# amathislab/BUCTD

Measured on AMD Instinct MI355X. Metric: images/sec (train) BUCTD-CoAM-W48 384x288, higher is better.
Workload: dtype f32 (3x3 convs: operands split exactly into 3 bf16 pieces, 6 bf16 MFMAs per product, fp32 accumulate - fp32-class); 1 GPU; BUCTD-CoAM-W48 (pose_hrnet_coam, ATT_MODULES [F,T,F,F], colored condition) 384x288 CrowdPose-14kpt full train step: fwd + JointsMSE + bwd + grad all-reduce + Adam + arg-max accuracy decode; global_batch=32, batch_per_gpu=32, input=N x 6 x 384 x 288 fp32, params=115581770, parallelism=dp1, hip_streams=4, conv_math=bf16x6, step_graph=False

## Files before the change

buctd_amd/csrc/conv3x3_wgrad.hip:

```cpp
#include "c3_common.h"

typedef __bf16 bf16x4 __attribute__((ext_vector_type(4)));

#define WG_MAX_SW 75
#define WG_PRO 96

template <int NP> struct WGeo;
template <> struct WGeo<2> { static constexpr int KB = 96; };
template <> struct WGeo<3> { static constexpr int KB = 64; };

struct WG3Args {
  const float* x;
  const float* dy;
  float* part;
  int N, H, W, Ci, Co;
  int SW, IB, P;
  int split_q, split_rem;
  const float* x_mean;
  const float* x_invstd;
  const float* x_gamma;
  const float* x_beta;
  int x_relu;
  unsigned ib_mul, ib_sh, sw_mul, sw_sh;
};

__device__ __forceinline__ int wg_fast_div(int n, unsigned mul, unsigned sh) {
  return (int)(__umulhi((unsigned)n, mul) >> sh);
}

typedef float wg_f32x2 __attribute__((ext_vector_type(2)));
typedef __bf16 wg_bf16x2 __attribute__((ext_vector_type(2)));
typedef unsigned wg_u32x2 __attribute__((ext_vector_type(2)));
template <int NP, int LO>
__device__ __forceinline__ void wg_split_store(unsigned char* row, int c, f32x4 v) {
  wg_f32x2 lo = {v.x, v.y}, hi = {v.z, v.w};
#pragma unroll
  for (int q = 0; q < NP; ++q) {
    const unsigned a = __builtin_bit_cast(unsigned, __builtin_convertvector(lo, wg_bf16x2));
    const unsigned b = __builtin_bit_cast(unsigned, __builtin_convertvector(hi, wg_bf16x2));
    *reinterpret_cast<wg_u32x2*>(row + q * LO + 2 * c) = (wg_u32x2){a, b};
    if (q + 1 < NP) {
      lo -= (wg_f32x2){__uint_as_float(a << 16), __uint_as_float(a & 0xffff0000u)};
      hi -= (wg_f32x2){__uint_as_float(b << 16), __uint_as_float(b & 0xffff0000u)};
    }
  }
}

__device__ __forceinline__ bf16x8 tr_frag(const unsigned char* p, int row_bytes) {
  typedef __attribute__((address_space(3))) bf16x4 lds_bf16x4;
  const bf16x4 a = __builtin_amdgcn_ds_read_tr16_b64_v4bf16((lds_bf16x4*)p);
  const bf16x4 b = __builtin_amdgcn_ds_read_tr16_b64_v4bf16((lds_bf16x4*)(p + 4 * row_bytes));
  return __builtin_shufflevector(a, b, 0, 1, 2, 3, 4, 5, 6, 7);
}

__device__ __forceinline__ bf16x8 tr_frag2(const unsigned char* p, const unsigned char* q) {
  typedef __attribute__((address_space(3))) bf16x4 lds_bf16x4;
  const bf16x4 a = __builtin_amdgcn_ds_read_tr16_b64_v4bf16((lds_bf16x4*)p);
  const bf16x4 b = __builtin_amdgcn_ds_read_tr16_b64_v4bf16((lds_bf16x4*)q);
  return __builtin_shufflevector(a, b, 0, 1, 2, 3, 4, 5, 6, 7);
}

__device__ __forceinline__ int ring_slot(int r, int ring) {
  return r - (r >= ring ? ring : 0);
}

#define WG_OOB 0x80000000u
template <int NP, int CF>
__device__ __forceinline__ void wg3_tile(const WG3Args& p, unsigned char* smem, int bxc, int byc, int z, int ncx, int nz) {
  constexpr int KB = WGeo<NP>::KB;
  constexpr int CH = CF * 16;
  constexpr int LO = CH * 2;
  constexpr int RS = (CH * 2 * NP) % 64 == 32 ? CH * 2 * NP : CH * 2 * NP + 32;
  constexpr int C4 = CH / 4;
  constexpr int PD = (KB * C4 + 255) / 256;
  constexpr int PP = (WG_PRO * C4 + 255) / 256;
  constexpr int NFR = 9 * CF;
  constexpr int NW = (NFR + 3) / 4;
  constexpr bool WHOLE = KB * C4 == PD * 256;

  const int R = KB + 2 * p.SW + 2;
  unsigned char* Dt = smem;
  unsigned char* Xt = smem + (size_t)KB * RS;
  float* bntab = reinterpret_cast<float*>(Xt + (size_t)R * RS);

  const int t = threadIdx.x, lane = t & 63;
  const int wave = __builtin_amdgcn_readfirstlane(t >> 6);
  const int t16 = lane & 15, g = lane >> 4;
  const int co0 = bxc * CH, ci0 = byc * CH;
  const int k_begin = (z * p.split_q + (z < p.split_rem ? z : p.split_rem)) * KB;
  int k_end = k_begin + (p.split_q + (z < p.split_rem ? 1 : 0)) * KB;
  if (k_end > p.P) k_end = p.P;
  const int halo = p.SW + 1;
  const int ci_lim = p.Ci - ci0;
  const bool x_bn = p.x_mean != nullptr;

  const __amdgpu_buffer_rsrc_t r_x = __builtin_amdgcn_make_buffer_rsrc(const_cast<float*>(p.x), 0, (unsigned)p.N * p.H * p.W * p.Ci * 4u, 0x00020000);
  const __amdgpu_buffer_rsrc_t r_d = __builtin_amdgcn_make_buffer_rsrc(const_cast<float*>(p.dy), 0, (unsigned)p.N * p.H * p.W * p.Co * 4u, 0x00020000);
  typedef unsigned wg_u32x4 __attribute__((ext_vector_type(4)));
  auto bload = [&](__amdgpu_buffer_rsrc_t r, unsigned off) -> f32x4 {
    return __builtin_bit_cast(f32x4, __builtin_amdgcn_raw_buffer_load_b128(r, off, 0, 0));
  };
  auto pos_offset = [&](int pp, int C, bool ok) -> unsigned {
    const int n = wg_fast_div(pp, p.ib_mul, p.ib_sh);
    const int rem = pp - n * p.IB;
    const int yy = wg_fast_div(rem, p.sw_mul, p.sw_sh);
    const int xx = rem - yy * p.SW;
    const bool real = ok & (pp >= 0) & (pp < p.P) & (n < p.N) & (yy >= 1) & (xx >= 1) & (xx <= p.W);
    return real ? (unsigned)(((n * p.H + yy - 1) * p.W + xx - 1) * C) * 4u : WG_OOB;
  };
  int srow[PD], sc4[PD];
#pragma unroll
  for (int q = 0; q < PD; ++q) {
    const int idx = t + 256 * q;
    srow[q] = idx / C4;
    sc4[q] = (idx - srow[q] * C4) * 4;
  }
  auto bn_in = [&](f32x4 v, int c, bool real) -> f32x4 {
    const f32x4 mu = *reinterpret_cast<const f32x4*>(bntab + c);
    const f32x4 sc = *reinterpret_cast<const f32x4*>(bntab + CH + c);
    const f32x4 be = *reinterpret_cast<const f32x4*>(bntab + 2 * CH + c);
#pragma unroll
    for (int j = 0; j < 4; ++j) {
      const float u = (v[j] - mu[j]) * sc[j] + be[j];
      const float w = p.x_relu ? fmaxf(u, 0.f) : u;
      v[j] = real ? w : 0.f;
    }
    return v;
  };

  f32x4 dreg[PD], xreg[PD];
  unsigned xoff[PD];
  auto load_d = [&](int k0) {
#pragma unroll
    for (int q = 0; q < PD; ++q) {
      const int pp = k0 + srow[q];
      dreg[q] = bload(r_d, pos_offset(pp, p.Co, (WHOLE || srow[q] < KB) & (pp < k_end)) + (unsigned)(co0 + sc4[q]) * 4u);
    }
  };
  auto load_x = [&](int rel0) {
#pragma unroll
    for (int q = 0; q < PD; ++q) {
      xoff[q] = pos_offset(k_begin - halo + rel0 + srow[q], p.Ci, (WHOLE || srow[q] < KB) & (sc4[q] < ci_lim));
      xreg[q] = bload(r_x, xoff[q] + (unsigned)(ci0 + sc4[q]) * 4u);
    }
  };
  auto store_d = [&]() {
#pragma unroll
    for (int q = 0; q < PD; ++q)
      if (WHOLE || srow[q] < KB) wg_split_store<NP, LO>(Dt + (size_t)srow[q] * RS, sc4[q], dreg[q]);
  };
  auto store_x = [&](int slot0) {
#pragma unroll
    for (int q = 0; q < PD; ++q)
      if (WHOLE || srow[q] < KB)
        wg_split_store<NP, LO>(Xt + (size_t)ring_slot(slot0 + srow[q], R) * RS, sc4[q],
                               x_bn ? bn_in(xreg[q], sc4[q], xoff[q] != WG_OOB) : xreg[q]);
  };

  f32x4 acc[CF][NW];
#pragma unroll
  for (int mf = 0; mf < CF; ++mf)
#pragma unroll
    for (int j = 0; j < NW; ++j) acc[mf][j] = (f32x4){0.f, 0.f, 0.f, 0.f};

  const int lane_row = g * 4 + (t16 >> 2), lane_col = (t16 & 3) * 8;
  const int lane_off = lane_row * RS + lane_col;

  if (x_bn) {
    for (int c = t; c < CH; c += 256) {
      const bool in = c < ci_lim;
      bntab[c] = in ? p.x_mean[ci0 + c] : 0.f;
      bntab[CH + c] = in ? p.x_invstd[ci0 + c] * p.x_gamma[ci0 + c] : 0.f;
      bntab[2 * CH + c] = in ? p.x_beta[ci0 + c] : 0.f;
    }
    __syncthreads();
  }
  if (k_begin < k_end) {
    const int pro = R - KB;
    for (int r0 = 0; r0 < pro; r0 += WG_PRO) {
      f32x4 preg[PP];
      unsigned poff[PP];
#pragma unroll
      for (int q = 0; q < PP; ++q) {
        const int idx = t + 256 * q;
        const int row = idx / C4, c4 = (idx - row * C4) * 4;
        poff[q] = pos_offset(k_begin - halo + r0 + row, p.Ci, (row < WG_PRO) & (r0 + row < pro) & (c4 < ci_lim));
        preg[q] = bload(r_x, poff[q] + (unsigned)(ci0 + c4) * 4u);
      }
#pragma unroll
      for (int q = 0; q < PP; ++q) {
        const int idx = t + 256 * q;
        const int row = idx / C4, c4 = (idx - row * C4) * 4;
        if (row < WG_PRO && r0 + row < pro)
          wg_split_store<NP, LO>(Xt + (size_t)(r0 + row) * RS, c4, x_bn ? bn_in(preg[q], c4, poff[q] != WG_OOB) : preg[q]);
      }
    }
    load_d(k_begin);
    load_x(pro);
  }
  int slot_new = R - KB;
  int slot_base = 0;
  int rel_next = R;
  const bool has_last = wave + 4 * (NW - 1) < NFR;
  for (int k0 = k_begin; k0 < k_end; k0 += KB) {
    __syncthreads();
    store_d();
    store_x(slot_new);
    if (k0 + KB < k_end) {
      load_d(k0 + KB);
      load_x(rel_next);
    }
    slot_new = ring_slot(slot_new + KB, R);
    rel_next += KB;
    __syncthreads();
    const unsigned ringb = (unsigned)R * RS;
    bf16x8 b[2][NP];
    auto read_b = [&](int ks, int j, bf16x8 (&dst)[NP]) {
      const int nf = wave + 4 * j;
      const int tap = nf / CF, cf = nf - tap * CF;
      const int shift = (tap / 3) * p.SW + tap % 3 + ks * 32;
      const int s = ring_slot(slot_base + shift, R);
      unsigned o0 = (unsigned)lane_off + (unsigned)(s * RS + cf * 32);
      o0 = o0 - ringb < o0 ? o0 - ringb : o0;
      unsigned o1 = o0 + 16 * RS;
      o1 = o1 - ringb < o1 ? o1 - ringb : o1;
      const unsigned char* q0 = Xt + o0;
      const unsigned char* q1 = Xt + o1;
#pragma unroll
      for (int pc = 0; pc < NP; ++pc) dst[pc] = tr_frag2(q0 + pc * LO, q1 + pc * LO);
    };
    read_b(0, 0, b[0]);
#pragma unroll
    for (int ks = 0; ks < KB / 32; ++ks) {
      bf16x8 a[NP][CF];
#pragma unroll
      for (int mf = 0; mf < CF; ++mf) {
        const unsigned char* q = Dt + (size_t)ks * 32 * RS + lane_off + mf * 32;
#pragma unroll
        for (int pc = 0; pc < NP; ++pc) a[pc][mf] = tr_frag(q + pc * LO, 4 * RS);
      }
#pragma unroll
      for (int j = 0; j < NW; ++j) {
        const int i = ks * NW + j;
        const bool more = i + 1 < (KB / 32) * NW;
        if (more) {
          const int jn = j + 1 < NW ? j + 1 : 0, ksn = j + 1 < NW ? ks : ks + 1;
          if (jn < NW - 1 || has_last) read_b(ksn, jn, b[(i + 1) & 1]);
        }
        if (j < NW - 1 || has_last) {
          bf16x8 (&bb)[NP] = b[i & 1];
#define WG_MMA(qa, qb)                                                                                      \
  _Pragma("unroll") for (int mf = 0; mf < CF; ++mf) acc[mf][j] =                                            \
      __builtin_amdgcn_mfma_f32_16x16x32_bf16(a[qa][mf], bb[qb], acc[mf][j], 0, 0, 0);
          if constexpr (NP == 3) {
            WG_MMA(2, 0) WG_MMA(0, 2) WG_MMA(1, 1) WG_MMA(1, 0) WG_MMA(0, 1) WG_MMA(0, 0)
          } else {
            WG_MMA(1, 0) WG_MMA(0, 1) WG_MMA(0, 0)
          }
#undef WG_MMA
        }
      }
    }
    slot_base = ring_slot(slot_base + KB, R);
  }

  {
    const size_t slab4 = (size_t)4 * NW * CF * 64;
    const size_t pair = (size_t)byc * ncx + bxc;
    f32x4* outp = reinterpret_cast<f32x4*>(p.part) + (pair * nz + z) * slab4;
#pragma unroll
    for (int j = 0; j < NW; ++j)
#pragma unroll
      for (int mf = 0; mf < CF; ++mf) {
        outp[((wave * NW + j) * CF + mf) * 64 + lane] = acc[mf][j];
      }
  }
}

template <int NP, int CF>
__global__ __launch_bounds__(256, 2) void conv3x3_wgrad_split_kernel(WG3Args p) {
  extern __shared__ __attribute__((aligned(16))) unsigned char smem[];
  wg3_tile<NP, CF>(p, smem, blockIdx.x, blockIdx.y, blockIdx.z, gridDim.x, gridDim.z);
}

#define WG3G_MAX 4
struct WG3Group {
  WG3Args conv[WG3G_MAX];
  int n;
  unsigned first[WG3G_MAX + 1];
  int ncx[WG3G_MAX], ncy[WG3G_MAX], nsplit[WG3G_MAX];
};
template <int NP, int CF>
__global__ __launch_bounds__(256, 2) void conv3x3_wgrad_group_kernel(WG3Group g_) {
  extern __shared__ __attribute__((aligned(16))) unsigned char smem[];
  const WG3Group& g = *(const WG3Group*)__builtin_amdgcn_kernarg_segment_ptr();
  int k = 0;
  while (k + 1 < g.n && blockIdx.x >= g.first[k + 1]) ++k;
  const unsigned lid = blockIdx.x - g.first[k], total = g.first[k + 1] - g.first[k];
  const unsigned xcd = lid & 7, idx = lid >> 3, per = total >> 3, rem = total & 7;
  const unsigned L = xcd < rem ? xcd * (per + 1) + idx : rem * (per + 1) + (xcd - rem) * per + idx;
  const unsigned pairs = (unsigned)(g.ncx[k] * g.ncy[k]);
  const unsigned z = L / pairs, pr = L - z * pairs;
  const unsigned byc = pr / (unsigned)g.ncx[k], bxc = pr - byc * (unsigned)g.ncx[k];
  wg3_tile<NP, CF>(g.conv[k], smem, (int)bxc, (int)byc, (int)z, g.ncx[k], g.nsplit[k]);
}

struct WG3Red { const float* part; float* out; int Ci, Co, nsplit, accumulate; };
template <int CF>
__device__ __forceinline__ void wg3_reduce_body(const WG3Red& a, f32x4 (&sm)[16][16], int bx, int nbx, int pair) {
  constexpr int NFR = 9 * CF;
  constexpr int NW = (NFR + 3) / 4;
  constexpr int SLAB = 4 * NW * CF * 64;
  const float* __restrict__ part = a.part;
  float* __restrict__ out = a.out;
  const int Ci = a.Ci, Co = a.Co, nsplit = a.nsplit, accumulate = a.accumulate;
  const int col = threadIdx.x & 15, zl = threadIdx.x >> 4;
  const int nco = Co / (CF * 16);
  const int co0 = (pair % nco) * CF * 16, ci0 = (pair / nco) * CF * 16;
  const f32x4* base = reinterpret_cast<const f32x4*>(part) + (size_t)pair * nsplit * SLAB;
  for (int e0 = bx * 16; e0 < SLAB; e0 += nbx * 16) {
    const int e = e0 + col;
    f32x4 s0 = (f32x4){0.f, 0.f, 0.f, 0.f}, s1 = s0, s2 = s0, s3 = s0;
    if (e < SLAB) {
      const f32x4* src = base + e;
      int zz = zl;
      for (; zz + 48 < nsplit; zz += 64) {
        s0 += src[(size_t)zz * SLAB];
        s1 += src[(size_t)(zz + 16) * SLAB];
        s2 += src[(size_t)(zz + 32) * SLAB];
        s3 += src[(size_t)(zz + 48) * SLAB];
      }
      for (; zz < nsplit; zz += 16) s0 += src[(size_t)zz * SLAB];
    }
    sm[zl][col] = (s0 + s1) + (s2 + s3);
    __syncthreads();
    if (zl == 0 && e < SLAB) {
      f32x4 sv = sm[0][col];
#pragma unroll
      for (int k = 1; k < 16; ++k) sv += sm[k][col];
      const int lane = e & 63, r = e >> 6;
      const int mf = r % CF, wj = r / CF, j = wj % NW, wv = wj / NW;
      const int nf = wv + 4 * j;
      if (nf < NFR) {
        const int tap = nf / CF, cf = nf - tap * CF;
        const int ci = ci0 + cf * 16 + (lane & 15);
        if (ci < Ci)
#pragma unroll
        for (int rg = 0; rg < 4; ++rg) {
          const int co = co0 + mf * 16 + (lane >> 4) * 4 + rg;
          float* dst = out + ((size_t)co * 9 + tap) * Ci + ci;
          *dst = accumulate ? *dst + sv[rg] : sv[rg];
        }
      }
    }
    __syncthreads();
  }
}
template <int CF>
__global__ __launch_bounds__(256) void wg3_reduce_kernel(WG3Red a) {
  __shared__ f32x4 sm[16][16];
  wg3_reduce_body<CF>(a, sm, blockIdx.x, gridDim.x, blockIdx.y);
}
struct WG3RedGroup {
  WG3Red r[WG3G_MAX];
  int n;
  unsigned first[WG3G_MAX + 1];
};
template <int CF>
__global__ __launch_bounds__(256) void wg3_reduce_group_kernel(WG3RedGroup g_) {
  __shared__ f32x4 sm[16][16];
  const WG3RedGroup& g = *(const WG3RedGroup*)__builtin_amdgcn_kernarg_segment_ptr();
  int k = 0;
  while (k + 1 < g.n && blockIdx.y >= g.first[k + 1]) ++k;
  wg3_reduce_body<CF>(g.r[k], sm, blockIdx.x, gridDim.x, (int)(blockIdx.y - g.first[k]));
}

struct WG3Plan { int CF, nsplit, q, rem; size_t lds; };

static void wg_magic(unsigned d, unsigned* mul, unsigned* sh) {
  unsigned l = 0;
  while ((1ull << l) < d) ++l;
  *mul = (unsigned)(((1ull << (31 + l)) + d - 1) / d);
  *sh = l - 1;
}

static bool wg3_plan(int np, int N, int H, int W, int Ci, int Co, WG3Plan* pl, int target = 0) {
  if ((np != 2 && np != 3) || c3_row_width(W) > WG_MAX_SW || H < 1 || W < 2) return false;
  if ((long)N * H * W * (Ci > Co ? Ci : Co) * 4 >= 2147483647L) return false;
  const int kb = np == 3 ? WGeo<3>::KB : WGeo<2>::KB;
  int cf;
  if (Ci % 48 == 0 && Co % 48 == 0) cf = 3;
  else if (Ci % 32 == 0 && Co % 32 == 0) cf = 2;
  else if (Co % 48 == 0 && Ci % 16 == 0 && Ci > 48) cf = 3;
  else return false;
  const int ch = cf * 16;
  const long P = (long)N * (H + 1) * c3_row_width(W) + c3_row_width(W);
  const long pairs = (long)(Co / ch) * ((Ci + ch - 1) / ch);
  long want = ((target > 0 ? target : (np == 3 ? 512 : 384)) + pairs - 1) / pairs;
  const long stages = (P + kb - 1) / kb;
  if (want > stages) want = stages;
  if (want < 1) want = 1;
  pl->CF = cf;
  pl->nsplit = (int)want;
  pl->q = (int)(stages / want);
  pl->rem = (int)(stages % want);
  int rs = ch * 2 * np;
  if (rs % 64 != 32) rs += 32;
  pl->lds = (size_t)(2 * kb + 2 * c3_row_width(W) + 2) * rs + (size_t)3 * ch * sizeof(float);
  return pl->lds <= 160 * 1024;
}

static size_t wg3_slab_floats(int cf) {
  return (size_t)4 * ((9 * cf + 3) / 4) * cf * 64 * 4;
}
static size_t wg3_ws_bytes(const WG3Plan& pl, int Ci, int Co) {
  const size_t pairs = (size_t)(Co / (pl.CF * 16)) * ((Ci + pl.CF * 16 - 1) / (pl.CF * 16));
  return pairs * pl.nsplit * wg3_slab_floats(pl.CF) * sizeof(float);
}

template <int NP, int CF>
static int wg3_launch(const WG3Args& a, const WG3Plan& pl, hipStream_t st) {
  static unsigned char attr_done[BUCTD_MAX_DEVICES] = {0};
  auto fn = conv3x3_wgrad_split_kernel<NP, CF>;
  const dim3 block(256);
  if (const int rc = buctd_raise_lds_limit(reinterpret_cast<const void*>(fn), 160 * 1024, attr_done, "conv3x3_wgrad (split bf16)"))
    return rc;
  dim3 grid(a.Co / (CF * 16), (a.Ci + CF * 16 - 1) / (CF * 16), pl.nsplit);
  hipLaunchKernelGGL(fn, grid, block, pl.lds, st, a);
  BUCTD_CHECK_LAUNCH("buctd_conv3x3_wgrad (split bf16)");
  return BUCTD_OK;
}

struct WG3InBn { const float* mean; const float* invstd; const float* gamma; const float* beta; int relu; };

static int wg3_fill(int np, int N, int H, int W, int Ci, int Co, const float* x, const float* dy, float* dw, void* workspace,
                    size_t workspace_bytes, const WG3InBn* x_bn, int target, WG3Args& a, WG3Plan& pl) {
  BUCTD_CHECK_ARG(x && dy && dw, "buctd_conv3x3_wgrad (split bf16): null tensor pointer");
  BUCTD_CHECK_ARG(wg3_plan(np, N, H, W, Ci, Co, &pl, target),
                  "buctd_conv3x3_wgrad (split bf16): unsupported shape N%d H%d W%d Ci%d Co%d", N, H, W, Ci, Co);
  const size_t need = wg3_ws_bytes(pl, Ci, Co);
  if (!workspace || workspace_bytes < need) {
    buctd_set_error("buctd_conv3x3_wgrad (split bf16): workspace %zu bytes < required %zu", workspace_bytes, need);
    return BUCTD_EWORKSPACE;
  }
  a.x = x; a.dy = dy; a.part = (float*)workspace;
  a.N = N; a.H = H; a.W = W; a.Ci = Ci; a.Co = Co;
  a.SW = c3_row_width(W); a.IB = (H + 1) * a.SW;
  const long P = (long)N * a.IB + a.SW;
  BUCTD_CHECK_ARG(P < 2147483647L, "buctd_conv3x3_wgrad (split bf16): tensor too large");
  a.P = (int)P;
  a.split_q = pl.q; a.split_rem = pl.rem;
  a.x_mean = a.x_invstd = a.x_gamma = a.x_beta = nullptr;
  a.x_relu = 0;
  if (x_bn && x_bn->mean) {
    BUCTD_CHECK_ARG(Ci % (pl.CF * 16) == 0, "buctd_conv3x3_wgrad: the fused input BatchNorm needs whole %d-channel chunks (Ci = %d)",
                    pl.CF * 16, Ci);
    BUCTD_CHECK_ARG(x_bn->invstd && x_bn->gamma && x_bn->beta, "buctd_conv3x3_wgrad: fused input BatchNorm needs all four arrays");
    a.x_mean = x_bn->mean; a.x_invstd = x_bn->invstd; a.x_gamma = x_bn->gamma; a.x_beta = x_bn->beta;
    a.x_relu = x_bn->relu;
  }
  wg_magic((unsigned)a.IB, &a.ib_mul, &a.ib_sh);
  wg_magic((unsigned)a.SW, &a.sw_mul, &a.sw_sh);
  return BUCTD_OK;
}

static int wg3_run(int np, int N, int H, int W, int Ci, int Co, const float* x, const float* dy, float* dw,
                   int accumulate, void* workspace, size_t workspace_bytes, void* stream, const WG3InBn* x_bn = nullptr) {
  WG3Plan pl;
  WG3Args a;
  int rc = wg3_fill(np, N, H, W, Ci, Co, x, dy, dw, workspace, workspace_bytes, x_bn, 0, a, pl);
  if (rc) return rc;
  hipStream_t st = (hipStream_t)stream;
  if (np == 3) rc = pl.CF == 3 ? wg3_launch<3, 3>(a, pl, st) : wg3_launch<3, 2>(a, pl, st);
  else rc = pl.CF == 3 ? wg3_launch<2, 3>(a, pl, st) : wg3_launch<2, 2>(a, pl, st);
  if (rc) return rc;
  const int pairs = (Co / (pl.CF * 16)) * ((Ci + pl.CF * 16 - 1) / (pl.CF * 16));
  const dim3 rgrid(ceil_div((long)(wg3_slab_floats(pl.CF) / 4), 16), pairs);
  const WG3Red ra{(const float*)workspace, dw, Ci, Co, pl.nsplit, accumulate};
  if (pl.CF == 3)
    hipLaunchKernelGGL(wg3_reduce_kernel<3>, rgrid, dim3(256), 0, st, ra);
  else
    hipLaunchKernelGGL(wg3_reduce_kernel<2>, rgrid, dim3(256), 0, st, ra);
  BUCTD_CHECK_LAUNCH("buctd_conv3x3_wgrad (split bf16, reduce)");
  return BUCTD_OK;
}

#define WG3_GROUP_PER_MEMBER 256
static int wg3_group_target(int n) { (void)n; return WG3_GROUP_PER_MEMBER; }

extern "C" size_t buctd_conv3x3_wgrad_bf16x6_group_workspace(int n, int N, int H, int W, int Ci, int Co) {
  WG3Plan pl;
  if (n < 1 || n > WG3G_MAX || !wg3_plan(3, N, H, W, Ci, Co, &pl, n > 1 ? wg3_group_target(n) : 0)) return 0;
  return wg3_ws_bytes(pl, Ci, Co);
}

extern "C" int buctd_conv3x3_wgrad_bf16x6_group(int n, const buctd_wg3_conv* convs, void* stream) {
  BUCTD_CHECK_ARG(n > 0 && n <= WG3G_MAX && convs, "buctd_conv3x3_wgrad_bf16x6_group: 1..%d convolutions", WG3G_MAX);
  if (n == 1) {
    const buctd_wg3_conv& c = convs[0];
    WG3InBn b{c.x_mean, c.x_invstd, c.x_gamma, c.x_beta, c.x_relu};
    return wg3_run(3, c.N, c.H, c.W, c.Ci, c.Co, c.x, c.dy, c.dw, c.accumulate, c.workspace, c.workspace_bytes, stream, &b);
  }
  WG3Group g;
  WG3RedGroup r;
  WG3Plan pl[WG3G_MAX];
  g.n = r.n = n;
  g.first[0] = r.first[0] = 0;
  size_t lds = 0;
  const int target = wg3_group_target(n);
  for (int k = 0; k < n; ++k) {
    const buctd_wg3_conv& c = convs[k];
    WG3InBn b{c.x_mean, c.x_invstd, c.x_gamma, c.x_beta, c.x_relu};
    const int rc = wg3_fill(3, c.N, c.H, c.W, c.Ci, c.Co, c.x, c.dy, c.dw, c.workspace, c.workspace_bytes, &b, target, g.conv[k], pl[k]);
    if (rc) return rc;
    BUCTD_CHECK_ARG(pl[k].CF == pl[0].CF, "buctd_conv3x3_wgrad_bf16x6_group: the convolutions must share the chunk width (48 or 32 channels)");
    const int ch = pl[k].CF * 16;
    g.ncx[k] = c.Co / ch;
    g.ncy[k] = (c.Ci + ch - 1) / ch;
    g.nsplit[k] = pl[k].nsplit;
    g.first[k + 1] = g.first[k] + (unsigned)(g.ncx[k] * g.ncy[k] * pl[k].nsplit);
    r.r[k] = WG3Red{(const float*)c.workspace, c.dw, c.Ci, c.Co, pl[k].nsplit, c.accumulate};
    r.first[k + 1] = r.first[k] + (unsigned)(g.ncx[k] * g.ncy[k]);
    if (pl[k].lds > lds) lds = pl[k].lds;
  }
  for (int k = n; k < WG3G_MAX; ++k) { g.first[k + 1] = g.first[n]; r.first[k + 1] = r.first[n]; g.ncx[k] = g.ncy[k] = g.nsplit[k] = 0; }
  hipStream_t st = (hipStream_t)stream;
  static unsigned char attr_done[2][BUCTD_MAX_DEVICES] = {{0}};
  const int cf = pl[0].CF;
  void (*fn)(WG3Group) = cf == 3 ? conv3x3_wgrad_group_kernel<3, 3> : conv3x3_wgrad_group_kernel<3, 2>;
  if (const int rc = buctd_raise_lds_limit(reinterpret_cast<const void*>(fn), 160 * 1024, attr_done[cf - 2], "buctd_conv3x3_wgrad_bf16x6_group"))
    return rc;
  hipLaunchKernelGGL(fn, dim3(g.first[n]), dim3(256), lds, st, g);
  BUCTD_CHECK_LAUNCH("buctd_conv3x3_wgrad_bf16x6_group");
  const dim3 rgrid(ceil_div((long)(wg3_slab_floats(cf) / 4), 16), r.first[n]);
  if (cf == 3) hipLaunchKernelGGL(wg3_reduce_group_kernel<3>, rgrid, dim3(256), 0, st, r);
  else hipLaunchKernelGGL(wg3_reduce_group_kernel<2>, rgrid, dim3(256), 0, st, r);
  BUCTD_CHECK_LAUNCH("buctd_conv3x3_wgrad_bf16x6_group (reduce)");
  return BUCTD_OK;
}

extern "C" int buctd_conv3x3_wgrad_bf16x6_group_workgroups(int n, const buctd_wg3_conv* convs) {
  BUCTD_CHECK_ARG(n > 0 && n <= WG3G_MAX && convs, "buctd_conv3x3_wgrad_bf16x6_group_workgroups: 1..%d convolutions", WG3G_MAX);
  long total = 0;
  for (int k = 0; k < n; ++k) {
    const buctd_wg3_conv& c = convs[k];
    WG3Plan pl;
    BUCTD_CHECK_ARG(wg3_plan(3, c.N, c.H, c.W, c.Ci, c.Co, &pl, n > 1 ? wg3_group_target(n) : 0),
                    "buctd_conv3x3_wgrad_bf16x6_group_workgroups: unsupported shape");
    const int ch = pl.CF * 16;
    total += (long)(c.Co / ch) * ((c.Ci + ch - 1) / ch) * pl.nsplit;
  }
  return (int)total;
}

static size_t wg3_workspace(int np, int N, int H, int W, int Ci, int Co) {
  WG3Plan pl;
  if (!wg3_plan(np, N, H, W, Ci, Co, &pl)) return 0;
  return wg3_ws_bytes(pl, Ci, Co);
}

extern "C" int buctd_conv3x3_wgrad_bf16x3_supported(int N, int H, int W, int Ci, int Co) {
  WG3Plan pl;
  return wg3_plan(2, N, H, W, Ci, Co, &pl) ? 1 : 0;
}
extern "C" size_t buctd_conv3x3_wgrad_bf16x3_workspace(int N, int H, int W, int Ci, int Co) {
  return wg3_workspace(2, N, H, W, Ci, Co);
}
extern "C" int buctd_conv3x3_wgrad_bf16x3(int N, int H, int W, int Ci, int Co, const float* x, const float* dy,
                                          float* dw, int accumulate, void* workspace, size_t workspace_bytes,
                                          void* stream) {
  return wg3_run(2, N, H, W, Ci, Co, x, dy, dw, accumulate, workspace, workspace_bytes, stream);
}
extern "C" int buctd_conv3x3_wgrad_bf16x6_plan(int N, int H, int W, int Ci, int Co, int* out) {
  WG3Plan pl;
  BUCTD_CHECK_ARG(out && wg3_plan(3, N, H, W, Ci, Co, &pl),
                  "buctd_conv3x3_wgrad_bf16x6_plan: unsupported shape N%d H%d W%d Ci%d Co%d", N, H, W, Ci, Co);
  out[0] = pl.CF; out[1] = pl.nsplit; out[2] = pl.q; out[3] = pl.rem;
  return BUCTD_OK;
}
extern "C" int buctd_conv3x3_wgrad_bf16x6_supported(int N, int H, int W, int Ci, int Co) {
  WG3Plan pl;
  return wg3_plan(3, N, H, W, Ci, Co, &pl) ? 1 : 0;
}
extern "C" size_t buctd_conv3x3_wgrad_bf16x6_workspace(int N, int H, int W, int Ci, int Co) {
  return wg3_workspace(3, N, H, W, Ci, Co);
}
extern "C" int buctd_conv3x3_wgrad_bf16x6(int N, int H, int W, int Ci, int Co, const float* x, const float* dy,
                                          float* dw, int accumulate, void* workspace, size_t workspace_bytes,
                                          void* stream) {
  return wg3_run(3, N, H, W, Ci, Co, x, dy, dw, accumulate, workspace, workspace_bytes, stream);
}
extern "C" int buctd_conv3x3_wgrad_bf16x6_bnin(int N, int H, int W, int Ci, int Co, const float* x, const float* dy,
                                               float* dw, int accumulate, const float* x_mean, const float* x_invstd,
                                               const float* x_gamma, const float* x_beta, int x_relu, void* workspace,
                                               size_t workspace_bytes, void* stream) {
  WG3InBn b{x_mean, x_invstd, x_gamma, x_beta, x_relu};
  return wg3_run(3, N, H, W, Ci, Co, x, dy, dw, accumulate, workspace, workspace_bytes, stream, &b);
}
```

Before: 510.7 images/s.

## Reshape wgrad split-K reduce: adaptive thread shape, double-buffered LDS, capped grid

The split-K reduction for the 3x3 weight-gradient kernel now picks its thread layout from the split count: 64 columns by 4 split lanes when nsplit is at most 4, otherwise 16 by 16. The LDS exchange buffer is double-buffered, which removes the trailing barrier in each iteration. The grid is capped near 8192 workgroups, with each workgroup walking several tiles, and the grouped launch becomes a flat 1D grid with per-member tile counts. The goal is less barrier overhead and fewer tiny workgroups in the reduce. In exchange, fewer workgroups may lower memory parallelism, and the indexing is more complex.

New measurement: 508.9 images/s. About the same (-0.4%).

```diff
diff --git a/buctd_amd/csrc/conv3x3_wgrad.hip b/buctd_amd/csrc/conv3x3_wgrad.hip
--- a/buctd_amd/csrc/conv3x3_wgrad.hip
+++ b/buctd_amd/csrc/conv3x3_wgrad.hip
@@ -305,21 +305,25 @@
   wg3_tile<NP, CF>(g.conv[k], smem, (int)bxc, (int)byc, (int)z, g.ncx[k], g.nsplit[k]);
 }
 
-struct WG3Red { const float* part; float* out; int Ci, Co, nsplit, accumulate; };
-template <int CF>
-__device__ __forceinline__ void wg3_reduce_body(const WG3Red& a, f32x4 (&sm)[16][16], int bx, int nbx, int pair) {
+enum { WG3R_64x4 = 0, WG3R_16x16 = 1 };
+struct WG3Red { const float* part; float* out; int Ci, Co, nsplit, accumulate, shape, nbx; };
+template <int CF, int E, int ZL>
+__device__ __forceinline__ void wg3_reduce_body(const WG3Red& a, f32x4* sm, int bx, int pair) {
+  static_assert(E * ZL == 256, "256 threads");
   constexpr int NFR = 9 * CF;
   constexpr int NW = (NFR + 3) / 4;
   constexpr int SLAB = 4 * NW * CF * 64;
   const float* __restrict__ part = a.part;
   float* __restrict__ out = a.out;
-  const int Ci = a.Ci, Co = a.Co, nsplit = a.nsplit, accumulate = a.accumulate;
-  const int col = threadIdx.x & 15, zl = threadIdx.x >> 4;
+  const int Ci = a.Ci, Co = a.Co, nsplit = a.nsplit, accumulate = a.accumulate, nbx = a.nbx;
+  const int col = threadIdx.x % E, zl = threadIdx.x / E;
   const int nco = Co / (CF * 16);
   const int co0 = (pair % nco) * CF * 16, ci0 = (pair / nco) * CF * 16;
   const f32x4* base = reinterpret_cast<const f32x4*>(part) + (size_t)pair * nsplit * SLAB;
-  for (int e0 = bx * 16; e0 < SLAB; e0 += nbx * 16) {
+  int buf = 0;
+  for (int e0 = bx * E; e0 < SLAB; e0 += nbx * E, buf ^= 1) {
     const int e = e0 + col;
+    f32x4* ex = sm + buf * 256;
     f32x4 s0 = (f32x4){0.f, 0.f, 0.f, 0.f}, s1 = s0, s2 = s0, s3 = s0;
     if (e < SLAB) {
       const f32x4* src = base + e;
@@ -332,12 +336,12 @@
       }
       for (; zz < nsplit; zz += 16) s0 += src[(size_t)zz * SLAB];
     }
-    sm[zl][col] = (s0 + s1) + (s2 + s3);
+    ex[zl * E + col] = (s0 + s1) + (s2 + s3);
     __syncthreads();
     if (zl == 0 && e < SLAB) {
-      f32x4 sv = sm[0][col];
-#pragma unroll
-      for (int k = 1; k < 16; ++k) sv += sm[k][col];
+      f32x4 sv = ex[col];
+#pragma unroll
+      for (int k = 1; k < ZL; ++k) sv += ex[k * E + col];
       const int lane = e & 63, r = e >> 6;
       const int mf = r % CF, wj = r / CF, j = wj % NW, wv = wj / NW;
       const int nf = wv + 4 * j;
@@ -353,13 +357,17 @@
         }
       }
     }
-    __syncthreads();
-  }
+  }
+}
+template <int CF>
+__device__ __forceinline__ void wg3_reduce_any(const WG3Red& a, f32x4* sm, int bx, int pair) {
+  if (a.shape == WG3R_64x4) wg3_reduce_body<CF, 64, 4>(a, sm, bx, pair);
+  else wg3_reduce_body<CF, 16, 16>(a, sm, bx, pair);
 }
 template <int CF>
 __global__ __launch_bounds__(256) void wg3_reduce_kernel(WG3Red a) {
-  __shared__ f32x4 sm[16][16];
-  wg3_reduce_body<CF>(a, sm, blockIdx.x, gridDim.x, blockIdx.y);
+  __shared__ f32x4 sm[2 * 256];
+  wg3_reduce_any<CF>(a, sm, blockIdx.x, blockIdx.y);
 }
 struct WG3RedGroup {
   WG3Red r[WG3G_MAX];
@@ -368,11 +376,12 @@
 };
 template <int CF>
 __global__ __launch_bounds__(256) void wg3_reduce_group_kernel(WG3RedGroup g_) {
-  __shared__ f32x4 sm[16][16];
+  __shared__ f32x4 sm[2 * 256];
   const WG3RedGroup& g = *(const WG3RedGroup*)__builtin_amdgcn_kernarg_segment_ptr();
   int k = 0;
-  while (k + 1 < g.n && blockIdx.y >= g.first[k + 1]) ++k;
-  wg3_reduce_body<CF>(g.r[k], sm, blockIdx.x, gridDim.x, (int)(blockIdx.y - g.first[k]));
+  while (k + 1 < g.n && blockIdx.x >= g.first[k + 1]) ++k;
+  const unsigned lid = blockIdx.x - g.first[k], nbx = (unsigned)g.r[k].nbx;
+  wg3_reduce_any<CF>(g.r[k], sm, (int)(lid % nbx), (int)(lid / nbx));
 }
 
 struct WG3Plan { int CF, nsplit, q, rem; size_t lds; };
@@ -418,6 +427,15 @@
   return pairs * pl.nsplit * wg3_slab_floats(pl.CF) * sizeof(float);
 }
 
+static int wg3_red_shape(int cf, int nsplit, WG3Red* r) {
+  r->shape = nsplit <= 4 ? WG3R_64x4 : WG3R_16x16;
+  return (int)(wg3_slab_floats(cf) / 4) / (r->shape == WG3R_64x4 ? 64 : 16);
+}
+#define WG3_RED_MAX_WORKGROUPS 8192
+static int wg3_red_walks(long tiles_in_launch) {
+  return (int)((tiles_in_launch + WG3_RED_MAX_WORKGROUPS - 1) / WG3_RED_MAX_WORKGROUPS);
+}
+
 template <int NP, int CF>
 static int wg3_launch(const WG3Args& a, const WG3Plan& pl, hipStream_t st) {
   static unsigned char attr_done[BUCTD_MAX_DEVICES] = {0};
@@ -475,8 +493,10 @@
   else rc = pl.CF == 3 ? wg3_launch<2, 3>(a, pl, st) : wg3_launch<2, 2>(a, pl, st);
   if (rc) return rc;
   const int pairs = (Co / (pl.CF * 16)) * ((Ci + pl.CF * 16 - 1) / (pl.CF * 16));
-  const dim3 rgrid(ceil_div((long)(wg3_slab_floats(pl.CF) / 4), 16), pairs);
-  const WG3Red ra{(const float*)workspace, dw, Ci, Co, pl.nsplit, accumulate};
+  WG3Red ra{(const float*)workspace, dw, Ci, Co, pl.nsplit, accumulate, 0, 0};
+  const int tiles = wg3_red_shape(pl.CF, pl.nsplit, &ra);
+  ra.nbx = ceil_div(tiles, wg3_red_walks((long)tiles * pairs));
+  const dim3 rgrid(ra.nbx, pairs);
   if (pl.CF == 3)
     hipLaunchKernelGGL(wg3_reduce_kernel<3>, rgrid, dim3(256), 0, st, ra);
   else
@@ -507,6 +527,8 @@
   g.n = r.n = n;
   g.first[0] = r.first[0] = 0;
   size_t lds = 0;
+  int rtiles[WG3G_MAX];
+  long rtotal = 0;
   const int target = wg3_group_target(n);
   for (int k = 0; k < n; ++k) {
     const buctd_wg3_conv& c = convs[k];
@@ -519,11 +541,12 @@
     g.ncy[k] = (c.Ci + ch - 1) / ch;
     g.nsplit[k] = pl[k].nsplit;
     g.first[k + 1] = g.first[k] + (unsigned)(g.ncx[k] * g.ncy[k] * pl[k].nsplit);
-    r.r[k] = WG3Red{(const float*)c.workspace, c.dw, c.Ci, c.Co, pl[k].nsplit, c.accumulate};
-    r.first[k + 1] = r.first[k] + (unsigned)(g.ncx[k] * g.ncy[k]);
+    r.r[k] = WG3Red{(const float*)c.workspace, c.dw, c.Ci, c.Co, pl[k].nsplit, c.accumulate, 0, 0};
+    rtiles[k] = wg3_red_shape(pl[k].CF, pl[k].nsplit, &r.r[k]);
+    rtotal += (long)rtiles[k] * g.ncx[k] * g.ncy[k];
     if (pl[k].lds > lds) lds = pl[k].lds;
   }
-  for (int k = n; k < WG3G_MAX; ++k) { g.first[k + 1] = g.first[n]; r.first[k + 1] = r.first[n]; g.ncx[k] = g.ncy[k] = g.nsplit[k] = 0; }
+  for (int k = n; k < WG3G_MAX; ++k) { g.first[k + 1] = g.first[n]; g.ncx[k] = g.ncy[k] = g.nsplit[k] = 0; }
   hipStream_t st = (hipStream_t)stream;
   static unsigned char attr_done[2][BUCTD_MAX_DEVICES] = {{0}};
   const int cf = pl[0].CF;
@@ -532,7 +555,13 @@
     return rc;
   hipLaunchKernelGGL(fn, dim3(g.first[n]), dim3(256), lds, st, g);
   BUCTD_CHECK_LAUNCH("buctd_conv3x3_wgrad_bf16x6_group");
-  const dim3 rgrid(ceil_div((long)(wg3_slab_floats(cf) / 4), 16), r.first[n]);
+  const int walks = wg3_red_walks(rtotal);
+  for (int k = 0; k < n; ++k) {
+    r.r[k].nbx = ceil_div(rtiles[k], walks);
+    r.first[k + 1] = r.first[k] + (unsigned)(g.ncx[k] * g.ncy[k] * r.r[k].nbx);
+  }
+  for (int k = n; k < WG3G_MAX; ++k) { r.r[k] = r.r[0]; r.first[k + 1] = r.first[n]; }
+  const dim3 rgrid(r.first[n]);
   if (cf == 3) hipLaunchKernelGGL(wg3_reduce_group_kernel<3>, rgrid, dim3(256), 0, st, r);
   else hipLaunchKernelGGL(wg3_reduce_group_kernel<2>, rgrid, dim3(256), 0, st, r);
   BUCTD_CHECK_LAUNCH("buctd_conv3x3_wgrad_bf16x6_group (reduce)");
```
